# line/open-universe

Hardware: AMD Instinct MI355X
Metric: real_time_factor (audio s / wall s), UNIVERSE++ 16 kHz 8-step enhance (higher is better)
Workload: dtype f32; 1 GPU; UNIVERSE++ 16 kHz, 8 diffusion steps, batch=1 utterance(s) of 4 s per GPU per step; network=PP16, n_diffusion_steps=8, batch_per_gpu=1, samples_per_utterance=64000, launches_per_enhance=414

## Files before the change

open-universe_amd/csrc/ou_api.cpp:

```cpp
#include <hip/hip_runtime.h>

#include <cmath>
#include <cstdio>
#include <cstdlib>
#include <cstring>
#include <map>
#include <string>
#include <vector>

#include "ou_variants.h"
#include "ou_walk.h"

using namespace ou;

namespace {
thread_local std::string g_last_error;
}

namespace ou {

int fail(ou_handle* h, int code, const std::string& msg) {
  if (h) h->err = msg;
  g_last_error = msg;
  return code;
}

bool launched(ou_handle* h, hipError_t e, const char* w) {
  h->n_launch++;
  if (e == hipSuccess) return true;
  fail(h, OU_EHIP, std::string("HIP error at ") + w + ": " + hipGetErrorString(e));
  return false;
}

}

namespace {

struct OptDesc {
  const char* key;
  int Options::*ip;
  double Options::*dp;
  bool experiments_only;
  const char* doc;
};
const OptDesc kOptions[] = {
    {"conv_direct", &Options::conv_direct, nullptr, false, "kernel generations the conv launcher may use (0 .. 5, ConvArgs::direct)"},
    {"split", &Options::split, nullptr, false, "-1 rule / 0 never / 1 wherever possible: conv_split_kernel (bf16-split operands)"},
    {"split_wino", &Options::split_wino, nullptr, false, "experiments build: 0 = the plain bf16-split kernel also where its minimal-filtering form would take the layer"},
    {"wino", &Options::wino, nullptr, false, "0: never the minimal-filtering (Winograd / Cook-Toom) kernel variants"},
    {"fuse", &Options::fuse, nullptr, false, "-1 cost model / 0 never / 2 / 3: depth of the fused ConvBlock body (conv_chain kernels)"},
    {"fuse_nc", &Options::fuse_nc, nullptr, false, "128 / 256: columns per tile of the fused ConvBlock body (0: launcher's choice)"},
    {"fuse_upfir", &Options::fuse_upfir, nullptr, false, "0: up-path anti-alias FIR always as its own pass"},
    {"rate_small", &Options::rate_small, nullptr, false, "0: outermost rate-change convs on the generic kernels (no rate_down / rate_up)"},
    {"preact", &Options::preact, nullptr, false, "0: every PReLU in its consumer's operand path (ConvArgs::out_act never set)"},
    {"unfuse64", &Options::unfuse64, nullptr, false, "1: 64-channel ConvBlock bodies as three split-K launches"},
    {"block3", &Options::block3, nullptr, false, "1: the three body convs of a deep-level ConvBlock in one launch (experiments build only)"},
    {"xcd_map", &Options::xcd_map, nullptr, false, "block -> tile mapping of the LDS-tiled conv kernel (-1: launcher's choice)"},
    {"d2_map", &Options::d2_map, nullptr, false, "block -> tile mapping of the wide-load split-K kernels (-1: launcher's choice)"},
    {"d2_tile_rule", &Options::d2_tile_rule, nullptr, false, "0: round 5's 64- vs 32-column rule of the wide-load split-K kernels (ignores that only 64-column tiles have minimal filtering)"},
    {"d2_wk", &Options::d2_wk, nullptr, false, "4 / 8: K slices of conv_direct2_kernel (0: launcher's rule)"},
    {"d4_fir", &Options::d4_fir, nullptr, false, "0: up convs with a fusable FIR stay on the first-generation fused kernel"},
    {"d4_short", &Options::d4_short, nullptr, false, "0: the 401-frame levels at batch 1 stay on the first-generation kernels"},
    {"d4_force", &Options::d4_force, nullptr, false, "10 TM + log2(WK): that conv_direct4 tile shape wherever a layer admits it"},
    {"tile_min", nullptr, &Options::tile_min, false, "wave tiles per SIMD from which the no-split-K kernels take a layer (< 0: 1.2)"},
    {"tile_prefetch", &Options::tile_prefetch, nullptr, false, "0: no LDS prefetch of the epilogue operand in conv_direct3_kernel"},
    {"deep_factor", &Options::deep_factor, nullptr, false, "blocks of 64 x 128 per CU up to which a layer counts as 'deep' (split-K kernels)"},
    {"mask_fused", &Options::mask_fused, nullptr, false, "ragged batches: 0 = a separate tail-mask launch after EVERY producer (reference form of the masks)"},
    {"gru_v", &Options::gru_v, nullptr, false, "2 ring kernel / 1 polling-wave kernel (experiments build)"},
    {"gru_bmax", &Options::gru_bmax, nullptr, false, "cap on the utterances per GRU launch (forces the chunked path)"},
    {"gru_upw", &Options::gru_upw, nullptr, false, "hidden units per workgroup of the ring kernel (0: from the batch size)"},
    {"gru_backoff", &Options::gru_backoff, nullptr, false, "poll back-off experiments of the ring kernel (0: none)"},
    {"gru_agent_stores", &Options::gru_agent, nullptr, false, "-1 handle's mode / 0 plain / 1 agent-scope publishes"},
    {"gru_dbg", &Options::gru_dbg, nullptr, false, "bit 0 no republish safety net, bit 1 system-scope publishes, bit 2 FAULT INJECTION (tests)"},
    {"gru_ts", &Options::gru_ts, nullptr, false, "1: per-wave cycle stamps of the GRU kernel into the end of the workspace (tuning)"},
    {"ts", &Options::ts, nullptr, false, "1: per-wave phase stamps in ou_bench_conv (tuning)"},
    {"trace", &Options::trace, nullptr, false, "1: one line per conv launch on stderr"},
    {"no_overlap", &Options::no_overlap, nullptr, false, "1: no side streams inside a call (every kernel alone on the device)"},
    {"ens_share", &Options::ens_share, nullptr, false, "ou_enhance_ensemble: 1 = conditioner once over the B inputs, its results replicated; 0 = over all E * B rows"},
    {"dbg", &Options::dbg, nullptr, true, "phase ablation switches of the conv kernels: WRONG results by design"},
    {"dbg_dec0", &Options::dbg_dec0_under_gru, nullptr, true, "first decoder block under the GRU: upper-bound measurement, WRONG results"},
};
constexpr int kNumOptions = (int)(sizeof(kOptions) / sizeof(kOptions[0]));
const OptDesc* find_option(const char* key) {
  for (int i = 0; i < kNumOptions; i++)
    if (std::strcmp(kOptions[i].key, key) == 0) return &kOptions[i];
  return nullptr;
}

}

extern "C" {

const char* ou_version(void) {
#ifdef OU_EXPERIMENTS
  return "libouniverse 0.2 (gfx950, fp32 MFMA) +experiments";
#else
  return "libouniverse 0.2 (gfx950, fp32 MFMA)";
#endif
}
const char* ou_last_error(const ou_handle* h) { return h ? h->err.c_str() : g_last_error.c_str(); }
const char* ou_packer_last_error(const ou_packer* p) { return p ? p->err.c_str() : g_last_error.c_str(); }

int ou_packer_create(const ou_config* cfg, ou_packer** out) {
  if (!cfg || !out) return fail(nullptr, OU_EINVAL, "null argument");
  auto* p = new ou_packer();
  std::string e = build_model(*cfg, p->m);
  if (!e.empty()) { delete p; return fail(nullptr, OU_ENOTIMPL, e); }
  *out = p;
  return OU_OK;
}

int ou_packer_set(ou_packer* p, const char* key, const float* data, const int64_t* shape, int32_t ndim) {
  if (!p || !key || !data || ndim < 0 || ndim > 8) return fail(nullptr, OU_EINVAL, "bad argument to ou_packer_set");
  HostTensor t;
  size_t n = 1;
  for (int i = 0; i < ndim; i++) { t.shape.push_back(shape[i]); n *= (size_t)shape[i]; }
  t.data.assign(data, data + n);
  p->sd[key] = std::move(t);
  return OU_OK;
}

int ou_packer_finish(ou_packer* p, const float** blob_host, size_t* nbytes) {
  if (!p || !blob_host || !nbytes) return fail(nullptr, OU_EINVAL, "null argument");
  int code = OU_OK;
  std::string e = pack_weights(p->m, p->sd, p->blob, code);
  if (!e.empty()) { p->err = e; g_last_error = e; return code; }
  *blob_host = p->blob.data();
  *nbytes = p->blob.size() * sizeof(float);
  return OU_OK;
}

void ou_packer_destroy(ou_packer* p) { delete p; }

int ou_packed_bytes(const ou_config* cfg, size_t* nbytes) {
  if (!cfg || !nbytes) return fail(nullptr, OU_EINVAL, "null argument");
  Model m;
  std::string e = build_model(*cfg, m);
  if (!e.empty()) return fail(nullptr, OU_ENOTIMPL, e);
  *nbytes = m.total_floats * sizeof(float);
  return OU_OK;
}

const char* ou_packer_plan_json(const ou_packer* p) { return p ? p->m.json.c_str() : ""; }
const char* ou_plan_json(const ou_handle* hc) {
  if (!hc) return "";
  ou_handle* h = const_cast<ou_handle*>(hc);
  std::string o = "\"options\": {";
  for (int i = 0; i < kNumOptions; i++) {
    const OptDesc& d = kOptions[i];
    char buf[96];
    if (d.ip) std::snprintf(buf, sizeof buf, "%s\"%s\": %d", i ? ", " : "", d.key, h->opt.*(d.ip));
    else std::snprintf(buf, sizeof buf, "%s\"%s\": %.9g", i ? ", " : "", d.key, h->opt.*(d.dp));
    o += buf;
  }
  o += "}";
  o += std::string(", \"noise_source\": \"") + (h->noise_src.on ? "counter" : "tensor") + "\"";
  {
    char buf[96];
    std::snprintf(buf, sizeof buf, ", \"norm\": \"%s\", \"zero_mean\": %d, \"norm_eps\": %.9g",
                  h->norm.norm == OU_NORM_MAX ? "max" : h->norm.norm == OU_NORM_2MAX ? "2-max" : "2", h->norm.zero_mean, h->norm.eps);
    o += buf;
  }
  const std::string& j = h->m.json;
  const size_t close = j.rfind('}');
  h->plan_with_options = close == std::string::npos ? "{" + o + "}" : j.substr(0, close) + ", " + o + j.substr(close);
  return h->plan_with_options.c_str();
}

int ou_set_normalization(ou_handle* h, int32_t norm_mode, int32_t zero_mean, float eps) {
  if (!h) return OU_EINVAL;
  if (norm_mode != OU_NORM_2 && norm_mode != OU_NORM_MAX && norm_mode != OU_NORM_2MAX)
    return fail(h, OU_EINVAL, "ou_set_normalization: norm_mode must be OU_NORM_2, OU_NORM_MAX or OU_NORM_2MAX");
  if (zero_mean != 0 && zero_mean != 1) return fail(h, OU_EINVAL, "ou_set_normalization: zero_mean must be 0 or 1");
  if (!(eps >= 0.f) || !std::isfinite(eps)) return fail(h, OU_EINVAL, "ou_set_normalization: eps must be finite and >= 0 (0: 1e-5)");
  h->norm.norm = norm_mode;
  h->norm.zero_mean = zero_mean;
  h->norm.eps = norm_mode == OU_NORM_2MAX && eps > 0.f ? eps : 1e-5f;
  return OU_OK;
}

int ou_set_option(ou_handle* h, const char* key, double value) {
  if (!h || !key) return fail(h, OU_EINVAL, "bad argument");
  const OptDesc* d = find_option(key);
  if (!d) return fail(h, OU_EMISSING, std::string("ou_set_option: no such option: ") + key);
#ifndef OU_EXPERIMENTS
  if (d->experiments_only && value != 0.0)
    return fail(h, OU_ENOTIMPL, std::string("ou_set_option: `") + key + "` makes calls return wrong results by design and exists in "
                "the experiments build (make EXPERIMENTS=1) only");
#endif
  if (d->ip) {
    if (value != std::floor(value) || std::fabs(value) > 2e9) return fail(h, OU_EINVAL, std::string("ou_set_option: `") + key + "` takes an integer");
    h->opt.*(d->ip) = (int)value;
  } else {
    h->opt.*(d->dp) = value;
  }
  h->trace = h->opt.trace != 0;
  h->overlap = h->opt.no_overlap == 0;
  return OU_OK;
}

int ou_get_option(const ou_handle* h, const char* key, double* value) {
  if (!h || !key || !value) return fail(const_cast<ou_handle*>(h), OU_EINVAL, "bad argument");
  const OptDesc* d = find_option(key);
  if (!d) return fail(const_cast<ou_handle*>(h), OU_EMISSING, std::string("ou_get_option: no such option: ") + key);
  *value = d->ip ? (double)(h->opt.*(d->ip)) : h->opt.*(d->dp);
  return OU_OK;
}

int ou_reset_options(ou_handle* h) {
  if (!h) return fail(h, OU_EINVAL, "bad argument");
  const std::string keep = h->opt.chain_ts;
  h->opt = Options();
  h->opt.chain_ts = keep;
  h->trace = false;
  h->overlap = true;
  return OU_OK;
}

int ou_option_count(void) { return kNumOptions; }
const char* ou_option_name(int32_t i) { return i >= 0 && i < kNumOptions ? kOptions[i].key : nullptr; }
const char* ou_option_doc(int32_t i) { return i >= 0 && i < kNumOptions ? kOptions[i].doc : nullptr; }
double ou_option_default(int32_t i) {
  if (i < 0 || i >= kNumOptions) return 0.0;
  const Options d;
  return kOptions[i].ip ? (double)(d.*(kOptions[i].ip)) : d.*(kOptions[i].dp);
}

int ou_set_stamp_layer(ou_handle* h, const char* block_name) {
  if (!h) return fail(h, OU_EINVAL, "bad argument");
  h->opt.chain_ts = block_name ? block_name : "";
  return OU_OK;
}

int ou_create(const ou_config* cfg, const void* weights_dev, size_t nbytes, int32_t device, ou_handle** out) {
  if (!cfg || !weights_dev || !out) return fail(nullptr, OU_EINVAL, "null argument");
  auto* h = new ou_handle();
  std::string e = build_model(*cfg, h->m);
  if (!e.empty()) { delete h; return fail(nullptr, OU_ENOTIMPL, e); }
  if (nbytes != h->m.total_floats * sizeof(float)) {
    size_t want = h->m.total_floats * sizeof(float);
    delete h;
    return fail(nullptr, OU_ESHAPE, "packed weight blob has " + std::to_string(nbytes) + " bytes, expected " + std::to_string(want));
  }
  int ndev = 0;
  hipError_t he = hipGetDeviceCount(&ndev);
  if (he != hipSuccess || ndev <= 0 || device < 0 || device >= ndev) {
    delete h;
    return fail(nullptr, OU_EHIP, "no HIP device available for ou_create (this library has no CPU path)");
  }
  hipDeviceProp_t prop;
  he = hipGetDeviceProperties(&prop, device);
  if (he != hipSuccess) { delete h; return fail(nullptr, OU_EHIP, hipGetErrorString(he)); }
  if (std::strncmp(prop.gcnArchName, "gfx950", 6) != 0) {
    std::string arch = prop.gcnArchName;
    delete h;
    return fail(nullptr, OU_EHIP, "libouniverse is built for gfx950 (MI355X) only; device is " + arch);
  }
  h->num_cu = prop.multiProcessorCount;
  h->trace = false;
  h->device = device;
  h->W = (const float*)weights_dev;
  (void)hipSetDevice(device);
  {
    std::vector<const ConvL*> all;
    auto addb = [&](const BlockL& b) { if (b.dir) all.push_back(&b.rc); all.push_back(&b.c1); all.push_back(&b.c2); all.push_back(&b.c3); };
    const Model& m = h->m;
    for (auto& b : m.s_enc) addb(b);
    for (auto& b : m.s_dec) addb(b);
    if (m.s_sandwich) { addb(m.s_cb1); addb(m.s_cb2); }
    addb(m.c_melblock);
    for (auto& b : m.c_enc) addb(b);
    for (auto& l : m.c_st) all.push_back(&l);
    addb(m.c_cb1); addb(m.c_cb2); addb(m.c_decin);
    for (auto& b : m.c_dec) addb(b);
// ... 305 lines not shown
```

open-universe_amd/csrc/ou_conv_chain.hip:

```cpp
#include "ou_kernels.h"
#include "ou_internal.h"
#include "ou_variants.h"
#include "ou_dev.h"

#include <cmath>
#include <cstdlib>
#include <type_traits>

namespace ou {

#ifdef OU_EXPERIMENTS
template <int MT, int NWV>
__global__ __launch_bounds__(64 * NWV) void conv_chain_kernel(ChainArgs p, int TN, int ntiles) {
  constexpr int C = 32 * MT, NTN = NWV / MT, NC = 32 * NTN, XS = NC + 4, NTH = 64 * NWV;
  constexpr int WSLOT = 96 * C;
  constexpr int MAXW = (WSLOT / 4 + NTH - 1) / NTH;
  constexpr int RPW = C / NWV, NCG = NC / 64;
  constexpr int U = 4;
  static_assert(NC % 64 == 0 && RPW * 4 <= 64 && C % NWV == 0, "input tile mapping");
  extern __shared__ __attribute__((aligned(16))) float smem[];
  float* bufA = smem;
  float* bufB = bufA + C * XS;
  float* Wb = bufB + C * XS;
  float* prm = Wb + 2 * WSLOT;
// ... 662 lines not shown
      const int ci = item / NCH, c = item - ci * NCH;
      const int ts = q0 * R + 4 * c - (fir ? R : 0);
      const int nwin = fir ? WIN : 4;
      const float* xr = xb + (size_t)ci * Tin;
      if (ts >= 0 && ts + nwin <= Tin) {
        if (!fir) {
          const f32x4 q = *reinterpret_cast<const f32x4u*>(xr + ts);
          v[u][0] = q.x; v[u][1] = q.y; v[u][2] = q.z; v[u][3] = q.w;
        } else {
#pragma unroll
          for (int i = 0; i < WIN; i += 2) {
            const f32x2 q = *reinterpret_cast<const f32x2*>(xr + ts + i);
            v[u][i] = q.x; v[u][i + 1] = q.y;
          }
        }
      } else {
#pragma unroll
        for (int i = 0; i < WIN; i++) {
          const int t = ts + i;
          v[u][i] = (i < nwin && t >= 0 && t < Tin) ? xr[t] : 0.f;
        }
      }
    }
    if (i0 == 0) {
#pragma unroll
      for (int ks = 0; ks < K2; ks++) {
        const int idx = 2 * ks + lhalf, ci = idx / R, tap = idx - ci * R;
        const int row = (((ci >> lck) * R + tap) << lck) + (ci & (CK - 1));
        a[ks] = p.w[(size_t)row * Mp + 32 * wm + l31];
      }
    }
#pragma unroll
    for (int u = 0; u < IB; u++) {
      const int item = tid + (i0 + u) * NT;
      const int ci = item / NCH, c = item - ci * NCH;
#pragma unroll
      for (int i = 0; i < WIN; i++) v[u][i] = (act && v[u][i] < 0.f) ? alpha * v[u][i] : v[u][i];
      f32x4 o;
      if (fir) {
#pragma unroll
        for (int j = 0; j < 4; j++) {
          float acc = 0.f;
#pragma unroll
          for (int i = 0; i <= 2 * R; i++) acc = fmaf(f[i], v[u][j + i], acc);
          o[j] = acc;
        }
      } else {
        o = f32x4{v[u][0], v[u][1], v[u][2], v[u][3]};
      }
      *reinterpret_cast<f32x4*>(&smem[ci * ROW + 4 * c]) = o;
    }
  }
  __syncthreads();
  floatx16 acc;
#pragma unroll
  for (int r = 0; r < 16; r++) acc[r] = 0.f;
  const float* bs = smem + (32 * wn + l31) * R;
#pragma unroll
  for (int ks = 0; ks < K2; ks++) {
    const int idx = 2 * ks + lhalf, ci = idx / R, tap = idx - ci * R;
    acc = __builtin_amdgcn_mfma_f32_32x32x2f32(a[ks], bs[ci * ROW + tap], acc, 0, 0, 0);
  }
  const int q = q0 + 32 * wn + l31;
  if (q < p.Nq) {
    const bool live = q < ragged_len(p.lens, b);
#pragma unroll
    for (int r = 0; r < 16; r++) {
      const int m = 32 * wm + (r & 3) + 8 * (r >> 2) + 4 * lhalf;
      if (m < p.M) p.y[((size_t)b * p.Cout + m) * p.Nq + q] = live ? acc[r] + p.bias[m] : 0.f;
    }
  }
  if (p.prof && tid == 0) atomicMin(p.prof + 16 + (blockIdx.x & 15), ~(unsigned long long)__builtin_amdgcn_s_memrealtime());
}

struct RateDownCfg {
  int R, M, Cin;
  void (*kern)(ConvArgs);
  int threads, bq;
};
static const RateDownCfg kRateDownCfgs[] = {
    {2, 64, 32, rate_down_kernel<2, 2, 2, 32>, 256, 64},
    {2, 96, 48, rate_down_kernel<2, 3, 1, 48>, 192, 32},
};
ConvPlan plan_rate_down(const ConvArgs& a, int) {
  if (a.up != 1 || a.stride != a.KW || a.pad != 0 || a.Tin != a.Nq * a.stride || a.add || a.film || a.res || a.in_scale)
    return no_plan(hipErrorNotSupported);
  if (a.fir && a.fir_len != 2 * a.stride + 1) return no_plan(hipErrorNotSupported);
  for (const RateDownCfg& c : kRateDownCfgs) {
    if (c.R != a.stride || c.M != a.M || c.Cin != a.Cin) continue;
    const size_t smem = (size_t)a.Cin * (c.bq * c.R + 4) * 4;
    return {hipSuccess, kVarRateDown + c.R, c.kern, dim3((a.Nq + c.bq - 1) / c.bq, a.B), dim3(c.threads), smem, a};
  }
  return no_plan(hipErrorNotSupported);
}

template <int R, int MT, int NWN, int K2>
__global__ __launch_bounds__(64 * MT * NWN) void rate_up_kernel(ConvArgs p) {
  constexpr int NW = MT * NWN, NT = 64 * NW, BF = 32 * NWN, UP = BF + 1;
  extern __shared__ __attribute__((aligned(16))) float smem[];
  const int tid = threadIdx.x, lane = tid & 63, lhalf = lane >> 5, l31 = lane & 31;
  const int wave = __builtin_amdgcn_readfirstlane(tid >> 6);
  const int wm = wave % MT, wn = wave / MT;
  const bool fir = p.fir != nullptr;
  const int H = fir ? 1 : 0, BV = BF - 2 * H;
  const int q0 = blockIdx.x * BV - H, b = blockIdx.y;
  if (p.prof && tid == 0) atomicMin(p.prof + (blockIdx.x & 15), (unsigned long long)__builtin_amdgcn_s_memrealtime());
  const int Tin = p.Tin, Mp = p.Mp;
  const int fq = q0 + 32 * wn + l31;
  const bool inside = fq >= 0 && fq < Tin;
  const float* xb = p.x + ((size_t)b * p.Cin + lhalf) * Tin + (inside ? fq : 0);
  float bx[K2], a[K2];
#pragma unroll
  for (int ks = 0; ks < K2; ks++) bx[ks] = inside ? xb[(size_t)2 * ks * Tin] : 0.f;
#pragma unroll
  for (int ks = 0; ks < K2; ks++) a[ks] = p.w[(size_t)(2 * ks + lhalf) * Mp + 32 * wm + l31];
  const float alpha = p.alpha_val;
  const bool act = p.act != 0;
  floatx16 acc;
#pragma unroll
  for (int r = 0; r < 16; r++) acc[r] = 0.f;
#pragma unroll
  for (int ks = 0; ks < K2; ks++) {
    const float x = bx[ks];
    acc = __builtin_amdgcn_mfma_f32_32x32x2f32(a[ks], (act && x < 0.f) ? alpha * x : x, acc, 0, 0, 0);
  }
#pragma unroll
  for (int r = 0; r < 16; r++) {
    const int row = 32 * wm + (r & 3) + 8 * (r >> 2) + 4 * lhalf;
    smem[row * UP + 32 * wn + l31] = inside ? acc[r] : 0.f;
  }
  __syncthreads();
  float f[2 * R + 1];
#pragma unroll
  for (int j = 0; j <= 2 * R; j++) f[j] = fir ? p.fir[j] : 0.f;
  const int Cout = p.Cout;
  const int rlen = ragged_len(p.lens, b);
  const int span = BV * R;
  const int total = Cout * span;
  if ((p.Tout & 3) == 0 && ((BF * R) & 3) == 0 && ((2 * R) & 3) == 0) {
    constexpr int QPT = (32 * MT / R * BF * R / 4 + NT - 1) / NT;
    f32x4 rs4[QPT];
    size_t idx4[QPT];
    int co4[QPT], tl4[QPT];
#pragma unroll
    for (int u = 0; u < QPT; u++) {
      const int e = 4 * (tid + u * NT);
      const int co = e / span, tl = e - co * span + H * R;
      const long t = (long)q0 * R + tl;
      const bool on = e < total && t < p.Tout;
      co4[u] = on ? co : -1; tl4[u] = tl;
      idx4[u] = on ? ((size_t)b * Cout + co) * p.Tout + (size_t)t : 0;
      rs4[u] = (on && p.res) ? *reinterpret_cast<const f32x4*>(p.res + idx4[u]) : f32x4{0.f, 0.f, 0.f, 0.f};
    }
#pragma unroll
    for (int u = 0; u < QPT; u++) {
      if (co4[u] < 0) continue;
      const float* urow = smem + (co4[u] * R) * UP;
      const float bi = p.bias[co4[u]];
      f32x4 o;
#pragma unroll
      for (int s4 = 0; s4 < 4; s4++) {
        const int tl = tl4[u] + s4;
        float v;
        if (fir) {
          int tau = tl - R, qf = tau / R, ph = tau - qf * R;
          v = 0.f;
#pragma unroll
          for (int j = 0; j <= 2 * R; j++) {
            v = fmaf(f[j], urow[ph * UP + qf], v);
            if (++ph == R) { ph = 0; qf++; }
// ... 84 lines not shown
```

open-universe_amd/csrc/ou_handle.h:

```cpp
#pragma once
#include <hip/hip_runtime.h>

#include <map>
#include <string>
#include <vector>

#include "../../include/ouniverse.h"
#include "../../include/ouniverse_tuning.h"
#include "ou_kernels.h"
#include "ou_model.h"

namespace ou {
constexpr int kMaxSteps = 256;
constexpr size_t kProfSlots = 32768;
constexpr float kInvSqrt2 = 0.70710678118654752440f;
constexpr size_t align256(size_t bytes) { return (bytes + 255) & ~size_t(255); }

struct TensorRef {
  size_t off;
  int C, T;
};
struct Options {
  int dbg = 0, xcd_map = -1, conv_direct = 5, fuse = -1, fuse_nc = 0, rate_small = 1, fuse_upfir = 1, block3 = 0, d4_fir = 1,
      d4_force = 0, d4_short = 1, d2_wk = 0, wino = 1, d2_map = -1, unfuse64 = 0, preact = 1;
  int gru_v = 2, gru_bmax = 0, gru_ts = 0, gru_upw = 0, gru_backoff = 0, gru_agent = -1, gru_dbg = 0;
  int split = -1;
  int dbg_dec0_under_gru = 0;
  int tile_prefetch = 1;
  int trace = 0, no_overlap = 0, ts = 0, deep_factor = 8, mask_fused = 1, split_wino = 1, d2_tile_rule = 1;
  int ens_share = 1;
  double tile_min = -1.0;
  std::string chain_ts;
};
}

struct ou_packer {
  ou::Model m;
  std::map<std::string, ou::HostTensor> sd;
  std::vector<float> blob;
  std::string err;
};

struct ou_handle {
  ou::Model m;
  const float* W = nullptr;
  int device = 0;
  int num_cu = 256;
  std::string err;
  std::map<std::string, ou::TensorRef> tensors;
  int n_launch = 0, n_conv = 0;
  int cond_B = 0, cond_T = 0;
  bool trace = false;
  ou::Options opt;
  ou::NormMode norm;
  std::string plan_with_options;
  int last_cfg = -1;
  long long* tstamps = nullptr;
  std::map<size_t, float> alphas;
  hipStream_t aux[3] = {nullptr, nullptr, nullptr};
  std::vector<hipEvent_t> events;
  size_t ev_used = 0;
  bool overlap = true;
  int force_cfg = -1, force_sc = 0;
  bool profile = false;
  struct ProfRec { double flops, bytes; int cfg; };
  std::vector<ProfRec> prof;
  size_t prof_used = 0;
  unsigned long long* prof_dev = nullptr;
  struct WsRec { const void* ws; size_t bytes; int B, T; };
  std::vector<WsRec> ws_ready;
  int gru_agent_stores = 0;
  int lanes = 1, lane = 0;
  int lane_max_b = 0;
  struct NoiseSource {
    bool on = false;
    unsigned long long seed = 0;
    std::vector<unsigned long long> streams;
    float* scratch = nullptr;
    size_t scratch_bytes = 0;
  } noise_src;
  double plane_per_sample = 0.0, wav_plane_per_sample = 0.0;
  bool ws_ok(const void* ws, size_t bytes, int B, int T) const {
    (void)T;
    for (const WsRec& r : ws_ready)
      if (r.ws == ws) return r.B == B && r.bytes <= bytes;
    return false;
  }
};

namespace ou {

int fail(ou_handle* h, int code, const std::string& msg);

struct Tensor {
  float* p = nullptr;
  int C = 0, T = 0;
};

bool launched(ou_handle* h, hipError_t e, const char* w);

}
```

open-universe_amd/csrc/ou_internal.h:

```cpp
#pragma once
#include <hip/hip_runtime.h>

#include "ou_kernels.h"

namespace ou {
hipError_t init_chain_kernels();
hipError_t init_direct3_kernels();
hipError_t init_block3_kernels();
hipError_t init_direct4_kernels();
hipError_t init_split_kernels();

struct ConvPlan {
  hipError_t status;
  int variant;
  void (*kern)(ConvArgs);
  dim3 grid, block;
  size_t smem;
  ConvArgs args;
};
inline ConvPlan no_plan(hipError_t why) { return ConvPlan{why, -1, nullptr, dim3(), dim3(), 0, ConvArgs()}; }
hipError_t launch_plan(const ConvPlan& p, hipStream_t stream);
ConvPlan plan_conv(const ConvArgs& a, int num_cu);
ConvPlan plan_conv_direct(const ConvArgs& a, int num_cu);
ConvPlan plan_conv_direct3(const ConvArgs& a, int num_cu);
ConvPlan plan_conv_direct4(const ConvArgs& a, int num_cu);
inline bool direct4_short_layer(const ConvArgs& a) { return a.Nq < 1024 && a.B < 4; }
ConvPlan plan_conv_direct4w(const ConvArgs& a, int num_cu);
ConvPlan plan_conv_split(const ConvArgs& a, int num_cu);
ConvPlan plan_rate_down(const ConvArgs& a, int num_cu = 0);
ConvPlan plan_rate_up(const ConvArgs& a, int num_cu = 0);
}
```

open-universe_amd/csrc/ou_kernels.h:

```cpp
#pragma once
#include <hip/hip_runtime.h>

#include <cstddef>
#include <cstdint>

namespace ou {

struct ConvArgs {
  const float* x = nullptr;
  const float* w = nullptr;
  const float* wd = nullptr;
  const float* wu = nullptr;
  const void* wsplit = nullptr;
  const void* wsplitw = nullptr;
  int split_wino = 1;
  const float* bias = nullptr;
  float* y = nullptr;
  const float* in_scale = nullptr;
  int act = 0;
  float alpha_val = 0.f;
  const float* add = nullptr;
  const float* film = nullptr;
  const float* res = nullptr;
  float add_scale = 1.f, res_scale = 1.f;
  int film_bstride = 0;
  int B = 1, Cin = 0, Tin = 0, Cout = 0, M = 0, Mp = 0, KW = 1, stride = 1, pad = 0, up = 1, CK = 2;
  int Nq = 0;
  int Tout = 0;
  unsigned magic_span[3] = {0, 0, 0};
  unsigned magic_up = 0;
  int SC = 1;
  int grid_n = 1, grid_m = 1;
  int xcd_map = 0;
  int force_cfg = -1, force_sc = 0;
  int force_xcd_map = -1;
  double tile_min = -1.0;
  int tile_prefetch = 1;
  int direct = 5;
  int d2_map = -1;
  int split = -1;
  int wino = 1;
  int d2_wk = 0;
  int d4_fir_unfused = 1;
  int d4_short = 1;
  int d4_force = 0;
  int d2_tile_rule = 1;
  int deep_factor = 8;
  int out_act = 0;
  float out_alpha = 1.f;
  const int* lens = nullptr;
  const float* fir = nullptr;
  int fir_len = 0;
  int tile_bm = 32, tile_bn = 0, tile_halo = 0;
  int dbg = 0;
  long long* tstamps = nullptr;
  unsigned long long* prof = nullptr;
};
hipError_t launch_conv(const ConvArgs& a, int num_cu, hipStream_t stream, int* cfg_out = nullptr);
hipError_t init_conv_kernels();
double direct3_tiles_per_simd(int M, int Nq, int B, int num_cu);

struct StepCoef {
  float w_in, sigma_net, w_skip, w_out, sig2, c1, s_next, beta;
};
enum OutMode { OUT_SCORE = 0, OUT_UPDATE = 1 };
hipError_t launch_in_conv(const float* x, const float* w, const float* bias, const StepCoef* coef, int coef_bstride,
                          float* y, int B, int C, int T, int KW, hipStream_t s, const int* lens = nullptr);
hipError_t launch_out_conv(const float* s, const float* w, const float* bias, const float* alphas, const float* x,
                           const float* noise, float* out, const StepCoef* coef, int coef_bstride, int edm,
                           int mode, int B, int C, int T, int KW, hipStream_t st, const int* lens = nullptr);

hipError_t launch_sigma_embed(const StepCoef* coef, int S, const float* params, int simple, int n_rff, int D,
                              float* g, hipStream_t st);
hipError_t launch_film(const float* g, const float* W, const float* b, float* film, int S, int rows, int D,
                       hipStream_t st);
struct CoefBlock { StepCoef c[64]; };
hipError_t launch_upload_coef(StepCoef* dst, const CoefBlock& blk, int n, hipStream_t st);

struct RowInfo { int t_raw, pad_left, t_pad, _r; };
struct NormMode {
  int norm = 0;
  int zero_mean = 1;
  float eps = 1e-5f;
  bool plain() const { return norm == 0 && zero_mean; }
  __host__ __device__ float gain(float level, float sd, float mx) const {
    if (norm == 1) return level / fmaxf(mx, eps);
    if (norm == 2) return fminf(level / fmaxf(sd, eps), 1.f / fmaxf(mx, eps));
    return level / fmaxf(sd, eps);
  }
};
constexpr int kMaxLenLevels = 8;
struct LevelSpec { int n = 0; int num[kMaxLenLevels]; int den[kMaxLenLevels]; };
struct RowBlock { int t_raw[64]; };
hipError_t launch_upload_rows(RowInfo* rows, int* lens, const RowBlock& blk, int n, int off, int B, int tot_ds,
                              const LevelSpec& lv, hipStream_t st);
hipError_t launch_mask_tail(float* y, const int* lens, int B, int C, int T, hipStream_t st);
hipError_t launch_gru_tail_fill(float* gx, const int* lens, int B, int H, int T, hipStream_t st);
hipError_t launch_pad_normalize_var(const float* mix, float* y, float* stats, const RowInfo* rows, int B, int T_raw_max,
                                    int T_pad_max, float level, const NormMode& nm, hipStream_t st);
hipError_t launch_post_var(const float* x, const float* stats, float* out, const RowInfo* rows, int B, int T_raw_max,
                           int T_pad_max, int keep_rms, int peak_guard, hipStream_t st);

hipError_t launch_pad_normalize(const float* mix, float* y, float* stats, int B, int T_raw, int T_pad, int pad_left,
                                float level, const NormMode& nm, hipStream_t st);
hipError_t launch_post(const float* x, const float* stats, float* out, int B, int T_raw, int T_pad, int pad_left,
                       int keep_rms, int peak_guard, hipStream_t st);
hipError_t launch_init_x(const float* noise, const float* base, float sigma, float* x, size_t n, hipStream_t st);

hipError_t launch_sampler_step(float* x, const float* score, const float* z, float c1, float c2, size_t n,
                               hipStream_t st);

hipError_t launch_stft_forward(const float* x, const float* win, float* out, int B, int T, int n_fft, int hop,
                               int type, float e, float factor, hipStream_t st);
hipError_t launch_stft_inverse(const float* spec, const float* win, float* frames, float* y, int B, int n_frames,
                               int n_fft, int hop, int type, float e, float factor, int length, hipStream_t st);

hipError_t launch_mel(const float* x, const float* win, const float* tw, const float* fb, float* mel, float* esum,
                      int B, int T, int n_fft, int hop, int pad_left, int n_freq, int n_mels, int L, hipStream_t st);
hipError_t launch_mel_scale(const float* esum, float* scale, int B, int L, hipStream_t st, const int* lens = nullptr);

struct SegGeom {
  long long T_raw, T_pad, pad_left;
  long long L, hop, overlap;
  long long n_win, n_entries;
};
struct SegRow { long long t_raw, T_pad, pad_left, n_win, first, frames; };
__host__ __device__ inline int seg_nb(long long T_raw) {
  const long long nb = (T_raw + (1ll << 18) - 1) >> 18;
  return (int)(nb < 1 ? 1 : nb > 1024 ? 1024 : nb);
}
struct SegRowsAlike {
  SegRow r;
  static constexpr bool zero_tail = false;
  __host__ __device__ SegRow row(long long) const { return r; }
  __host__ __device__ long long stride() const { return r.t_raw; }
// ... 252 lines not shown
```

open-universe_amd/csrc/ou_walk.cpp:

```cpp
#include "ou_walk.h"
#include "ou_internal.h"
#include "ou_variants.h"

#include <algorithm>
#include <cmath>
#include <cstdio>

#include "../../include/ouniverse_tuning.h"

namespace ou {

void Runner::wait_for(hipStream_t from, hipStream_t to, const char* w_record, const char* w_wait) {
  if (dry || !ok()) return;
  hipEvent_t e = next_event();
  if (!e) { herr = hipErrorOutOfMemory; where = "event"; return; }
  launch(w_record, [&] { return hipEventRecord(e, from); });
  launch(w_wait, [&] { return hipStreamWaitEvent(to, e, 0); });
}

ConvArgs Runner::conv_args(const ConvL& L, const Tensor& in, const Tensor& out, const Epi& e) {
  ConvArgs a;
  a.x = in.p; a.w = W(L.w_off); a.bias = W(L.b_off); a.y = out.p;
  if (L.KWP) { a.wd = W(L.wd_off); a.wu = W(L.wu_off); }
  if (L.ws_on) a.wsplit = W(L.ws_off);
  if (L.wsw_on) a.wsplitw = W(L.wsw_off);
  a.split = env.split; a.split_wino = env.split_wino;
  a.in_scale = e.in_scale;
  a.act = (L.act && e.act) ? 1 : 0;
  a.alpha_val = a.act ? h->alphas[L.a_off] : 0.f;
  a.add = e.add; a.add_scale = e.add_scale;
  a.film = e.film; a.film_bstride = e.film_bstride;
  a.res = e.res; a.res_scale = e.res_scale;
  if (e.out_act && !e.fir && !e.rate_down && !e.rate_up) { a.out_act = 1; a.out_alpha = e.out_alpha; }
  if (e.fir && !e.rate_down) { a.fir = e.fir; a.fir_len = e.fir_len; a.bias = e.fir_bias; }
  if (e.rate_down) { a.fir = e.fir; a.fir_len = e.fir ? e.fir_len : 0; }
  a.B = B; a.Cin = L.Cin; a.Tin = in.T; a.Cout = L.Cout; a.M = L.M; a.Mp = L.Mp; a.KW = L.KW;
  a.stride = L.stride; a.pad = L.pad; a.up = L.up; a.CK = L.CK; a.Nq = conv_nq(L, in.T); a.Tout = conv_tout(L, in.T);
  a.force_cfg = h->force_cfg; a.force_sc = h->force_sc;
  a.dbg = env.dbg; a.force_xcd_map = env.xcd_map; a.direct = env.conv_direct; a.d4_fir_unfused = env.d4_fir; a.d4_force = env.d4_force; a.d4_short = env.d4_short; a.deep_factor = env.deep_factor; a.d2_tile_rule = env.d2_tile_rule; a.d2_wk = env.d2_wk; a.wino = env.wino; a.d2_map = env.d2_map;
  a.tile_min = env.tile_min; a.tile_prefetch = env.tile_prefetch;
  a.tstamps = h->tstamps;
  if (ragged && env.mask_fused && !e.no_mask) a.lens = lens_of(a.Tout);
  return a;
}

Runner::ConvOut Runner::conv(const ConvL& L, const Tensor& in, const std::string& name, const Epi& e, const Tensor* dst) {
  ConvOut o;
  o.out = dst ? *dst : alloc(name, L.Cout, conv_tout(L, in.T));
  if (dry || !ok()) return o;
  ConvArgs a = conv_args(L, in, o.out, e);
  a.prof = prof_open(2.0 * L.M * (double)a.Nq * L.Cin * L.KW * B,
                     4.0 * ((double)B * ((double)L.Cin * in.T + (double)L.Cout * a.Tout) + (double)L.M * L.Cin * L.KW), -1);
  ConvPlan p = e.rate_down ? plan_rate_down(a) : e.rate_up ? plan_rate_up(a) : plan_conv(a, h->num_cu);
  if (!e.rate_down && !e.rate_up) {
    if (p.status == hipErrorNotSupported && a.out_act) {
      a.out_act = 0;
      p = plan_conv(a, h->num_cu);
    }
    o.stored_act = a.out_act != 0;
    if (p.status == hipErrorNotSupported && e.fir) {
      prof_drop(a.prof);
      o.supported = false;
      return o;
    }
  }
  const int cfg = p.variant;
  const hipError_t le = launch_plan(p, st);
  launch(L.name.c_str(), [le] { return le; });
  prof_close(a.prof, cfg);
  h->last_cfg = cfg;
  if (!e.no_mask && !(a.lens && conv_masks_rows(cfg))) mask(o.out);
  if (h->trace)
    std::fprintf(stderr, "OU_TRACE conv %-64s cfg=%d M=%d Nq=%d K=%d(Cin=%d KW=%d CK=%d) stride=%d up=%d B=%d MFLOP=%.1f\n",
                 name.c_str(), cfg, L.M, a.Nq, L.Cin * L.KW, L.Cin, L.KW, L.CK, L.stride, L.up, B,
                 2.0 * L.M * a.Nq * L.Cin * L.KW * B * 1e-6);
  h->n_conv++;
  return o;
}


ConvArgs Runner::rate_probe(const ConvL& rc, int Tin) {
  ConvArgs a;
  a.up = rc.up; a.stride = rc.stride; a.KW = rc.KW; a.pad = rc.pad; a.Tin = Tin;
  a.Nq = conv_nq(rc, Tin); a.Tout = conv_tout(rc, Tin); a.M = rc.M; a.Cout = rc.Cout; a.Cin = rc.Cin;
  a.fir = (rc.fir_mode == 1 || rc.fir_mode == 2) ? W(rc.fir_off) : nullptr; a.fir_len = rc.fir_len;
  return a;
}

Tensor Runner::up_path(const BlockL& Bk, const Tensor& hin, const std::string& nm, const float* res) {
  if (Bk.dir != 2) return hin;
  const ConvL& rc = Bk.rc;
  Epi e;
  e.res = res; e.res_scale = kInvSqrt2;
  if (rc.fir_mode == 2) { e.fir = W(rc.fir_off); e.fir_len = rc.fir_len; e.fir_bias = W(rc.fbias_off); }
  if ((rc.fir_mode == 0 || rc.fir_mode == 2) && env.rate_small != 0 && plan_rate_up(rate_probe(rc, hin.T)).status == hipSuccess) {
    e.rate_up = true;
    return conv(rc, hin, nm + ".up", e).out;
  }
  if (rc.fir_mode != 2) return conv(rc, hin, nm + ".up", e).out;
  const Tensor u = alloc(nm + ".upc", rc.Cout, hin.T * rc.up);
  const Tensor hu = alloc(nm + ".up", u.C, u.T);
  if (env.fuse_upfir != 0 && conv(rc, hin, nm + ".up", e, &hu).supported) return hu;
  conv(rc, hin, nm + ".upc", Epi(), &u);
  launch_masked("fir(up)", hu.p, hu.C, hu.T, [&](const int* ln) {
    return launch_fir(u.p, W(rc.fir_off), rc.fir_len, 0.f, 0, W(rc.fbias_off), res, kInvSqrt2, hu.p, B, u.C, u.T, st, ln);
  });
  return hu;
}

ChainArgs Runner::chain_args(const BlockL& Bk, int depth, const Tensor& hu, const Tensor& c1, const Tensor& v, const Epi& e1,
                             bool need_c1) {
  ChainArgs ca;
  ca.depth = depth; ca.B = B; ca.C = Bk.C; ca.T = hu.T; ca.Mp = Bk.c1.Mp;
  ca.x = depth == 3 ? hu.p : c1.p;
  ca.y = v.p; ca.res = hu.p; ca.res_scale = kInvSqrt2;
  if (depth == 3) {
    ca.add = e1.add; ca.add_scale = e1.add_scale; ca.film = e1.film; ca.film_bstride = e1.film_bstride;
    ca.c1_out = need_c1 ? c1.p : nullptr;
  }
  const ConvL* ls[3] = {&Bk.c1, &Bk.c2, &Bk.c3};
  for (int s2 = 0; s2 < depth; s2++) {
    const ConvL& L = *ls[3 - depth + s2];
    if (!L.act || L.stride != 1 || L.up != 1 || L.Cin != Bk.C || L.Cout != Bk.C || L.pad != (L.KW - 1) / 2 || L.Mp != Bk.c1.Mp)
      ca.depth = 0;
    ChainConv& c = ca.cv[s2];
    c.w = W(L.w_off); c.bias = W(L.b_off); c.alpha = L.act ? h->alphas[L.a_off] : 0.f; c.KW = L.KW; c.CK = L.CK;
    if (L.KWP) c.wu = W(L.wu_off);
  }
  ca.force_nc = env.fuse_nc;
  ca.wino = env.wino && env.conv_direct >= 5;
  ca.lens = lens_of(hu.T);
  return ca;
}
int Runner::plan_chain(const BlockL& Bk, const Tensor& hu, const Tensor& c1, const Tensor& v, const Epi& e1, bool need_c1) {
  const int T = hu.T;
  if (env.fuse == 0) return 0;
// ... 409 lines not shown
```

Before: 615.5 x_realtime.

## Add persistent strip-walking kernel for small rate-down convs with register prefetch

Adds a persistent rate_stream_kernel for the outermost stride-2 rate-down conv (32->64 channels). Each block walks several strips, prefetches the next strip's input windows into registers while the MFMA of the current one runs, and double-buffers the LDS tile. Weights stay in registers across strips. It is enabled by a rule that fires at batch <=2 when there are enough strips per CU, which covers the default batch=1 4 s case. Risks are lower occupancy from one block per CU, and a single layer having only a small share of the 414 launches.

```diff
diff --git a/open-universe_amd/csrc/ou_api.cpp b/open-universe_amd/csrc/ou_api.cpp
--- a/open-universe_amd/csrc/ou_api.cpp
+++ b/open-universe_amd/csrc/ou_api.cpp
@@ -52,6 +52,7 @@
     {"fuse_nc", &Options::fuse_nc, nullptr, false, "128 / 256: columns per tile of the fused ConvBlock body (0: launcher's choice)"},
     {"fuse_upfir", &Options::fuse_upfir, nullptr, false, "0: up-path anti-alias FIR always as its own pass"},
     {"rate_small", &Options::rate_small, nullptr, false, "0: outermost rate-change convs on the generic kernels (no rate_down / rate_up)"},
+    {"rate_stream", &Options::rate_stream, nullptr, false, "0 never / 1 rule / 2 wherever legal: the strip walk of the small-K rate-change convs (rate_stream_kernel)"},
     {"preact", &Options::preact, nullptr, false, "0: every PReLU in its consumer's operand path (ConvArgs::out_act never set)"},
     {"unfuse64", &Options::unfuse64, nullptr, false, "1: 64-channel ConvBlock bodies as three split-K launches"},
     {"block3", &Options::block3, nullptr, false, "1: the three body convs of a deep-level ConvBlock in one launch (experiments build only)"},
@@ -190,6 +191,8 @@
 #endif
   if (d->ip) {
     if (value != std::floor(value) || std::fabs(value) > 2e9) return fail(h, OU_EINVAL, std::string("ou_set_option: `") + key + "` takes an integer");
+    if (d->ip == &Options::rate_stream && (value < 0 || value > 2))
+      return fail(h, OU_EINVAL, std::string("ou_set_option: `") + key + "` is 0 (off), 1 (rule) or 2 (wherever legal)");
     h->opt.*(d->ip) = (int)value;
   } else {
     h->opt.*(d->dp) = value;
diff --git a/open-universe_amd/csrc/ou_conv_chain.hip b/open-universe_amd/csrc/ou_conv_chain.hip
--- a/open-universe_amd/csrc/ou_conv_chain.hip
+++ b/open-universe_amd/csrc/ou_conv_chain.hip
@@ -768,10 +768,14 @@
     {2, 64, 32, rate_down_kernel<2, 2, 2, 32>, 256, 64},
     {2, 96, 48, rate_down_kernel<2, 3, 1, 48>, 192, 32},
 };
-ConvPlan plan_rate_down(const ConvArgs& a, int) {
+ConvPlan plan_rate_down(const ConvArgs& a, int num_cu) {
   if (a.up != 1 || a.stride != a.KW || a.pad != 0 || a.Tin != a.Nq * a.stride || a.add || a.film || a.res || a.in_scale)
     return no_plan(hipErrorNotSupported);
   if (a.fir && a.fir_len != 2 * a.stride + 1) return no_plan(hipErrorNotSupported);
+  {
+    const ConvPlan s = plan_rate_stream_down(a, num_cu);
+    if (s.status == hipSuccess) return s;
+  }
   for (const RateDownCfg& c : kRateDownCfgs) {
     if (c.R != a.stride || c.M != a.M || c.Cin != a.Cin) continue;
     const size_t smem = (size_t)a.Cin * (c.bq * c.R + 4) * 4;
diff --git a/open-universe_amd/csrc/ou_conv_stream.hip b/open-universe_amd/csrc/ou_conv_stream.hip
--- /dev/null
+++ b/open-universe_amd/csrc/ou_conv_stream.hip
@@ -0,0 +1,169 @@
+#include "ou_kernels.h"
+#include "ou_internal.h"
+#include "ou_variants.h"
+#include "ou_dev.h"
+
+namespace ou {
+
+template <int R, int K2, int NT, int NCH, int ITEMS>
+__device__ __forceinline__ void stream_load_windows(float (&v)[ITEMS][4 + 2 * R], const float* __restrict__ xb, int Tin, int t0,
+                                                    bool fir, int tid) {
+  constexpr int WIN = 4 + 2 * R;
+#pragma unroll
+  for (int u = 0; u < ITEMS; u++) {
+    const int item = tid + u * NT;
+    const int ci = item / NCH, c = item - ci * NCH;
+    const int ts = t0 + 4 * c - (fir ? R : 0);
+    const int nwin = fir ? WIN : 4;
+    const float* xr = xb + (size_t)ci * Tin;
+    if (ts >= 0 && ts + nwin <= Tin) {
+      if (!fir) {
+        const f32x4 q = *reinterpret_cast<const f32x4u*>(xr + ts);
+        v[u][0] = q.x; v[u][1] = q.y; v[u][2] = q.z; v[u][3] = q.w;
+#pragma unroll
+        for (int i = 4; i < WIN; i++) v[u][i] = 0.f;
+      } else {
+#pragma unroll
+        for (int i = 0; i < WIN; i += 2) {
+          const f32x2 q = *reinterpret_cast<const f32x2*>(xr + ts + i);
+          v[u][i] = q.x; v[u][i + 1] = q.y;
+        }
+      }
+    } else {
+#pragma unroll
+      for (int i = 0; i < WIN; i++) {
+        const int t = ts + i;
+        v[u][i] = (i < nwin && t >= 0 && t < Tin) ? xr[t] : 0.f;
+      }
+    }
+  }
+}
+
+template <int R, int MT, int NWQ, int K2>
+__global__ __launch_bounds__(64 * MT * NWQ) void rate_stream_kernel(ConvArgs p) {
+  constexpr int NW = MT * NWQ, NT = 64 * NW, BQ = 32 * NWQ, SP = BQ * R, ROW = SP + 4, NCH = SP / 4;
+  constexpr int CIN = 2 * K2 / R, ITEMS = CIN * NCH / NT, WIN = 4 + 2 * R;
+  static_assert(SP % 4 == 0 && (2 * K2) % R == 0 && R % 2 == 0, "runs of 4 samples, whole channels, even windows");
+  static_assert(CIN * NCH % NT == 0, "items per thread");
+  extern __shared__ __attribute__((aligned(16))) float smem[];
+  const int tid = threadIdx.x, lane = tid & 63, lhalf = lane >> 5, l31 = lane & 31;
+  const int wave = __builtin_amdgcn_readfirstlane(tid >> 6);
+  const int wm = wave % MT, wq = wave / MT;
+  if (p.prof && tid == 0) atomicMin(p.prof + (blockIdx.x & 15), (unsigned long long)__builtin_amdgcn_s_memrealtime());
+  const int Cin = p.Cin, Tin = p.Tin, Mp = p.Mp, CK = p.CK, lck = 31 - __clz(CK), Nq = p.Nq;
+  const int nsq = p.grid_n, total = nsq * p.B, step = gridDim.x;
+  const bool fir = p.fir != nullptr;
+  float f[2 * R + 1];
+#pragma unroll
+  for (int j = 0; j <= 2 * R; j++) f[j] = fir ? p.fir[j] : 0.f;
+  const float alpha = p.alpha_val;
+  const bool act = p.act != 0;
+  int s = blockIdx.x;
+  float v[ITEMS][WIN];
+  {
+    const int b = s / nsq;
+    stream_load_windows<R, K2, NT, NCH, ITEMS>(v, p.x + (size_t)b * Cin * Tin, Tin, (s - b * nsq) * BQ * R, fir, tid);
+  }
+  float a[K2];
+#pragma unroll
+  for (int ks = 0; ks < K2; ks++) {
+    const int idx = 2 * ks + lhalf, ci = idx / R, tap = idx - ci * R;
+    const int row = (((ci >> lck) * R + tap) << lck) + (ci & (CK - 1));
+    a[ks] = p.w[(size_t)row * Mp + 32 * wm + l31];
+  }
+  const int m = 32 * wm + l31;
+  const bool mrow = m < p.M;
+  const float bm = mrow ? p.bias[m] : 0.f;
+  const bool vec = (Nq & 3) == 0;
+  int buf = 0;
+#pragma unroll 1
+  for (; s < total; s += step, buf ^= 1) {
+    const int b = s / nsq, q0 = (s - b * nsq) * BQ;
+    float* xf = smem + buf * (CIN * ROW);
+#pragma unroll
+    for (int u = 0; u < ITEMS; u++) {
+      const int item = tid + u * NT;
+      const int ci = item / NCH, c = item - ci * NCH;
+#pragma unroll
+      for (int i = 0; i < WIN; i++) v[u][i] = (act && v[u][i] < 0.f) ? alpha * v[u][i] : v[u][i];
+      f32x4 o;
+      if (fir) {
+#pragma unroll
+        for (int j = 0; j < 4; j++) {
+          float acc = 0.f;
+#pragma unroll
+          for (int i = 0; i <= 2 * R; i++) acc = fmaf(f[i], v[u][j + i], acc);
+          o[j] = acc;
+        }
+      } else {
+        o = f32x4{v[u][0], v[u][1], v[u][2], v[u][3]};
+      }
+      *reinterpret_cast<f32x4*>(&xf[ci * ROW + 4 * c]) = o;
+    }
+    __syncthreads();
+    const int sn = s + step;
+    if (sn < total) {
+      const int bn = sn / nsq;
+      stream_load_windows<R, K2, NT, NCH, ITEMS>(v, p.x + (size_t)bn * Cin * Tin, Tin, (sn - bn * nsq) * BQ * R, fir, tid);
+    }
+    floatx16 acc;
+#pragma unroll
+    for (int r = 0; r < 16; r++) acc[r] = 0.f;
+    const float* as = xf + (32 * wq + l31) * R;
+#pragma unroll
+    for (int ks = 0; ks < K2; ks++) {
+      const int idx = 2 * ks + lhalf, ci = idx / R, tap = idx - ci * R;
+      acc = __builtin_amdgcn_mfma_f32_32x32x2f32(as[ci * ROW + tap], a[ks], acc, 0, 0, 0);
+    }
+    const int rlen = ragged_len(p.lens, b);
+    float* yr = p.y + ((size_t)b * p.Cout + m) * Nq;
+#pragma unroll
+    for (int j = 0; j < 4; j++) {
+      const int qj = q0 + 32 * wq + 8 * j + 4 * lhalf;
+      f32x4 o = f32x4{acc[4 * j] + bm, acc[4 * j + 1] + bm, acc[4 * j + 2] + bm, acc[4 * j + 3] + bm};
+      o = ragged_mask4(o, qj, rlen);
+      if (!mrow || qj >= Nq) continue;
+      if (vec) {
+        *reinterpret_cast<f32x4*>(yr + qj) = o;
+      } else {
+#pragma unroll
+        for (int e = 0; e < 4; e++)
+          if (qj + e < Nq) yr[qj + e] = o[e];
+      }
+    }
+  }
+  if (p.prof && tid == 0) atomicMin(p.prof + 16 + (blockIdx.x & 15), ~(unsigned long long)__builtin_amdgcn_s_memrealtime());
+}
+
+#ifndef OU_STREAM_BLOCKS_PER_CU
+#define OU_STREAM_BLOCKS_PER_CU 1
+#endif
+
+struct RateStreamCfg {
+  int R, M, Cin;
+  void (*kern)(ConvArgs);
+  int threads, bq;
+};
+static const RateStreamCfg kRateStreamDownCfgs[] = {
+    {2, 64, 32, rate_stream_kernel<2, 2, 2, 32>, 256, 64},
+};
+
+ConvPlan plan_rate_stream_down(const ConvArgs& a, int num_cu) {
+  if (a.rate_stream == 0) return no_plan(hipErrorNotSupported);
+  const int cus = num_cu > 0 ? num_cu : 256;
+  for (const RateStreamCfg& c : kRateStreamDownCfgs) {
+    if (c.R != a.stride || c.M != a.M || c.Cin != a.Cin) continue;
+    const int nsq = (a.Nq + c.bq - 1) / c.bq;
+    const long total = (long)nsq * a.B;
+    if (total > 0x3fffffffL) return no_plan(hipErrorNotSupported);
+    if (a.rate_stream == 1 && !(a.B <= 2 && 2 * total >= 3L * cus)) return no_plan(hipErrorNotSupported);
+    const long blocks = total < (long)OU_STREAM_BLOCKS_PER_CU * cus ? total : (long)OU_STREAM_BLOCKS_PER_CU * cus;
+    const size_t smem = (size_t)2 * a.Cin * (c.bq * c.R + 4) * 4;
+    ConvPlan p = {hipSuccess, kVarRateDown + c.R + 1, c.kern, dim3((unsigned)blocks), dim3(c.threads), smem, a};
+    p.args.grid_n = nsq;
+    return p;
+  }
+  return no_plan(hipErrorNotSupported);
+}
+
+}
diff --git a/open-universe_amd/csrc/ou_handle.h b/open-universe_amd/csrc/ou_handle.h
--- a/open-universe_amd/csrc/ou_handle.h
+++ b/open-universe_amd/csrc/ou_handle.h
@@ -28,6 +28,7 @@
   int dbg_dec0_under_gru = 0;
   int tile_prefetch = 1;
   int trace = 0, no_overlap = 0, ts = 0, deep_factor = 8, mask_fused = 1, split_wino = 1, d2_tile_rule = 1;
+  int rate_stream = 1;
   int ens_share = 1;
   double tile_min = -1.0;
   std::string chain_ts;
diff --git a/open-universe_amd/csrc/ou_internal.h b/open-universe_amd/csrc/ou_internal.h
--- a/open-universe_amd/csrc/ou_internal.h
+++ b/open-universe_amd/csrc/ou_internal.h
@@ -29,4 +29,5 @@
 ConvPlan plan_conv_split(const ConvArgs& a, int num_cu);
 ConvPlan plan_rate_down(const ConvArgs& a, int num_cu = 0);
 ConvPlan plan_rate_up(const ConvArgs& a, int num_cu = 0);
+ConvPlan plan_rate_stream_down(const ConvArgs& a, int num_cu);
 }
diff --git a/open-universe_amd/csrc/ou_kernels.h b/open-universe_amd/csrc/ou_kernels.h
--- a/open-universe_amd/csrc/ou_kernels.h
+++ b/open-universe_amd/csrc/ou_kernels.h
@@ -51,6 +51,7 @@
   const int* lens = nullptr;
   const float* fir = nullptr;
   int fir_len = 0;
+  int rate_stream = 0;
   int tile_bm = 32, tile_bn = 0, tile_halo = 0;
   int dbg = 0;
   long long* tstamps = nullptr;
diff --git a/open-universe_amd/csrc/ou_walk.cpp b/open-universe_amd/csrc/ou_walk.cpp
--- a/open-universe_amd/csrc/ou_walk.cpp
+++ b/open-universe_amd/csrc/ou_walk.cpp
@@ -38,7 +38,7 @@
   a.stride = L.stride; a.pad = L.pad; a.up = L.up; a.CK = L.CK; a.Nq = conv_nq(L, in.T); a.Tout = conv_tout(L, in.T);
   a.force_cfg = h->force_cfg; a.force_sc = h->force_sc;
   a.dbg = env.dbg; a.force_xcd_map = env.xcd_map; a.direct = env.conv_direct; a.d4_fir_unfused = env.d4_fir; a.d4_force = env.d4_force; a.d4_short = env.d4_short; a.deep_factor = env.deep_factor; a.d2_tile_rule = env.d2_tile_rule; a.d2_wk = env.d2_wk; a.wino = env.wino; a.d2_map = env.d2_map;
-  a.tile_min = env.tile_min; a.tile_prefetch = env.tile_prefetch;
+  a.tile_min = env.tile_min; a.tile_prefetch = env.tile_prefetch; a.rate_stream = env.rate_stream;
   a.tstamps = h->tstamps;
   if (ragged && env.mask_fused && !e.no_mask) a.lens = lens_of(a.Tout);
   return a;
@@ -51,7 +51,7 @@
   ConvArgs a = conv_args(L, in, o.out, e);
   a.prof = prof_open(2.0 * L.M * (double)a.Nq * L.Cin * L.KW * B,
                      4.0 * ((double)B * ((double)L.Cin * in.T + (double)L.Cout * a.Tout) + (double)L.M * L.Cin * L.KW), -1);
-  ConvPlan p = e.rate_down ? plan_rate_down(a) : e.rate_up ? plan_rate_up(a) : plan_conv(a, h->num_cu);
+  ConvPlan p = e.rate_down ? plan_rate_down(a, h->num_cu) : e.rate_up ? plan_rate_up(a) : plan_conv(a, h->num_cu);
   if (!e.rate_down && !e.rate_up) {
     if (p.status == hipErrorNotSupported && a.out_act) {
       a.out_act = 0;
```

Result: no change. 617.0 x_realtime, median of 3 (+0.2%).
